# kamisli-icpl/LLICTI

Measured on AMD Instinct MI355X. Metric: MPix/s encode+decode, higher is better.
Workload: dtype f32; 1 GPU; 24x768x512 uniform-noise RGB per GPU, container xauto15 -> xrans20, seed-1337 weights; BASELINE.json configs[2]; batch_per_gpu=24, height=512, width=768, container=xauto15, container_written=xrans20

## Files before the change

__graft_entry__.py:

```python
import os
import subprocess
import sys

ROOT = os.path.dirname(os.path.abspath(__file__))
if ROOT not in sys.path:
    sys.path.insert(0, ROOT)


def build() -> None:
    from llicti_amd import _lib
    so = _lib.build()
    L = _lib.lib()
    assert L.llicti_version()
    _lib.build_probe()
    from oracle import oracle as orc
    orc.build()
    import llicti_amd
    from llicti_amd.graphs.models.LLICTI_nets import LLICTI
    from llicti_amd.agents.llicti_agent import LLICTIAgent
    print("built", so)


def smoke() -> None:
    import numpy as np
    import torch
    assert torch.cuda.is_available(), "smoke() needs cuda:0"
    from llicti_amd.codec import HipCodec, container_to_bytestream_list
    from llicti_amd.config import default_config
    from llicti_amd.graphs.models.LLICTI_nets import LLICTI
    from llicti_amd.weights import pack_state_dict
    from oracle import oracle as orc

    torch.manual_seed(1337)
    model = LLICTI(default_config()).to("cuda:0").eval()
    rgb = np.random.default_rng(0).integers(0, 256, size=(3, 96, 160), dtype=np.uint8)
    x = torch.from_numpy(rgb.astype(np.float32) / np.float32(255)).unsqueeze(0).to("cuda:0")
    bl, _ = model.compress(x)
    model.codec().poison_workspace()
    x_reco = model.decompres(bl, torch.device("cuda:0"))
    assert np.array_equal((x_reco * 255).round().to(torch.uint8).cpu().numpy()[0], rgb), "lossless round trip failed"
    ref = orc.encode_image(rgb, orc.Weights(pack_state_dict(model.state_dict())))
    assert ref == bl, "HIP bitstream differs from the CPU oracle"
    nbytes = sum(len(s) for row in bl for s in row)
    from llicti_amd.codec import MODE_RANS
    codec = model.codec()
    dev_rgb = torch.from_numpy(rgb[None]).to("cuda:0")
    W_o = orc.Weights(pack_state_dict(model.state_dict()))
    sizes = []
    for M, wide in ((10, 2), (10, 1), (8, 0)):
        mode = MODE_RANS(M, wide=wide)
        cont, seg = codec.encode(dev_rgb, mode=mode)
        codec.check()
        got = container_to_bytestream_list(cont[0].cpu().numpy(), seg[0].cpu().numpy())
        assert got == orc.encode_image_rans(rgb, W_o, M, wide), "HIP rANS container differs from the CPU oracle"
        codec.poison_workspace()
        rec = codec.decode(cont, seg, 96, 160, mode=mode)
        codec.check()
        assert torch.equal(rec, dev_rgb), "rANS container: lossless round trip failed"
        sizes.append(int(seg.sum().item()))
    from llicti_amd.codec import MODE_RANS_AUTO, name_of_mode
    cont, seg = codec.encode(dev_rgb, mode=MODE_RANS_AUTO(3))
    codec.check()
    picked = codec.container_modes(cont)[0]
    assert container_to_bytestream_list(cont[0].cpu().numpy(), seg[0].cpu().numpy()) == orc.encode_image_rans(rgb, W_o, 3, 2, auto=True), "auto stream count: HIP container differs from the CPU oracle"
    codec.poison_workspace()
    assert torch.equal(codec.decode(cont, seg, 96, 160, mode=picked), dev_rgb), "auto stream count: lossless round trip failed"
    codec.check()
    small = np.random.default_rng(1).integers(0, 256, size=(3, 67, 93), dtype=np.uint8)
    mode = MODE_RANS(2, wide=2)
    flat = torch.from_numpy(np.concatenate([rgb.reshape(-1), small.reshape(-1)])).to("cuda:0")
    cont, seg = codec.encode_v(flat, [96, 67], [160, 93], mode)
    codec.check()
    for b, img in enumerate((rgb, small)):
        assert container_to_bytestream_list(cont[b].cpu().numpy(), seg[b].cpu().numpy()) == orc.encode_image_rans(img, W_o, 2, 2), "mixed-size batch differs from the CPU oracle"
    codec.poison_workspace()
    assert torch.equal(codec.decode_v(cont, seg, [96, 67], [160, 93], mode), flat), "mixed-size batch: lossless round trip failed"
    codec.check()
    print(f"smoke ok: 96x160 image, {nbytes} bytes (reference format) / {sizes[0]} bytes (rANS, 10 xwide v4 streams) / {sizes[1]} bytes "
          f"(10 wide streams) / {sizes[2]} bytes (8 streams), xauto3 -> {name_of_mode(picked)}, and a 96x160 + 67x93 batch in one call: all bit-exact with the oracle, lossless")

if __name__ == "__main__":
    build()
    if len(sys.argv) > 1 and sys.argv[1] == "smoke":
        smoke()
```

llicti_amd/_lib.py:

```python
from __future__ import annotations

import ctypes as C
import os
import subprocess

_HERE = os.path.dirname(os.path.abspath(__file__))
ROOT = os.path.dirname(_HERE)
SO_PATH = os.environ.get("LLICTI_HIP_SO") or os.path.join(_HERE, "libllicti_hip.so")
_CSRC = os.path.join(_HERE, "csrc")
SOURCES = [os.path.join(_CSRC, "llicti_hip.hip")] + sorted(os.path.join(_CSRC, f) for f in os.listdir(_CSRC) if f.endswith(".hpp")) + \
          [os.path.join(ROOT, "include", "llicti_hip.h")]
HIPCC_FLAGS = ["--offload-arch=gfx950", "-O3", "-std=c++17", "-ffp-contract=off", "-fPIC", "-shared",
               "-Wno-unused-value"]

OK, EINVAL, EHIP, ENOWEIGHTS, ENOSPACE, EFORMAT, ENODEVICE = 0, -1, -2, -3, -4, -5, -6


class LlictiError(RuntimeError):
    def __init__(self, code, msg):
        super().__init__(f"llicti_hip error {code}: {msg}")
        self.code = code


def build(force: bool = False) -> str:
    stale = force or not os.path.exists(SO_PATH) or any(
        os.path.getmtime(s) > os.path.getmtime(SO_PATH) for s in SOURCES)
    if stale:
        hipcc = os.environ.get("HIPCC", "/opt/rocm/bin/hipcc")
        cmd = [hipcc] + HIPCC_FLAGS + ["-o", SO_PATH, SOURCES[0]]
        subprocess.check_call(cmd)
    return SO_PATH


PROBE_SRC = os.path.join(ROOT, "tests", "numerics_probe.hip")
PROBE_PATH = os.path.join(ROOT, "tests", "numerics_probe")


def build_probe(force: bool = False) -> str:
    deps = [PROBE_SRC, os.path.join(_CSRC, "numerics.hpp")]
    stale = force or not os.path.exists(PROBE_PATH) or any(os.path.getmtime(s) > os.path.getmtime(PROBE_PATH) for s in deps)
    if stale:
        hipcc = os.environ.get("HIPCC", "/opt/rocm/bin/hipcc")
        flags = [f for f in HIPCC_FLAGS if f not in ("-shared", "-fPIC")]
        subprocess.check_call([hipcc] + flags + ["-o", PROBE_PATH, PROBE_SRC])
    return PROBE_PATH


_lib = None
_vp, _i, _l, _sz =C.c_void_p, C.c_int, C.c_long, C.c_size_t
VIEW_GROUPS_MAX = 16
RECORD_CHUNK = 32768


class ViewGroup(C.Structure):
    _fields_ = [("d_out", C.c_void_p), ("dtype", C.c_int), ("Ho", C.c_int), ("Wo", C.c_int), ("antialias", C.c_int), ("n", C.c_int),
                ("image", C.c_void_p), ("y0", C.c_void_p), ("x0", C.c_void_p), ("hs", C.c_void_p), ("ws", C.c_void_p), ("flip", C.c_void_p)]


class TensorOpts(C.Structure):
    _fields_ = [("layout", C.c_int), ("pad_mode", C.c_int), ("fill_space", C.c_int), ("fill", C.c_float * 3)]


_SIGS = {
    "llicti_last_error": (C.c_char_p, []),
    "llicti_version": (C.c_char_p, []),
    "llicti_create": (_i, [C.POINTER(_vp), _i]),
    "llicti_destroy": (_i, [_vp]),
    "llicti_set_band_weights": (_i, [_vp, _i, _i] + [_vp] * 6),
    "llicti_set_model": (_i, [_vp, _i, _i]),
    "llicti_workspace_bytes_ctx": (_sz, [_vp, _i, _vp, _vp, _vp, _i]),
    "llicti_max_container_bytes_ctx": (_sz, [_vp, _i, _i]),
    "llicti_level_geom": (_i, [_i, _i, _i, _i] + [C.POINTER(_i)] * 8),
    "llicti_lift_u8": (_i, [_vp, _vp, _i, _i, _i, _vp, _vp, _vp, _vp]),
    "llicti_unlift_u8": (_i, [_vp, _vp, _i, _i, _i, _vp, _vp]),
    "llicti_band_params_f32": (_i, [_vp, _vp, _i, _i, _i, _i, _i, _vp, _vp]),
    "llicti_lift_train_f32": (_i, [_vp, _vp, _i, _i, _i, _vp, _vp]),
    "llicti_selfinfo_f32": (_i, [_vp, _vp, _vp, _i, _i, _i, _i, _i, _vp, _vp]),
    "llicti_cdf_u16": (_i, [_vp, _vp, _vp, _vp, _i, _i, _i, _i, _i, _i, _vp, _i, _vp]),
    "llicti_cdf_pairs_u32": (_i, [_vp, _vp, _vp, _vp, _i, _i, _i, _i, _i, _vp, _vp]),
    "llicti_ac_encode_u16cdf": (_i, [_vp, _vp, _i, _i, _vp, _i, _l, _vp, _l, _vp, _vp]),
    "llicti_ac_decode_u16cdf": (_i, [_vp, _vp, _i, _i, _vp, _l, _vp, _i, _l, _vp, _vp]),
    "llicti_workspace_bytes": (_sz, [_i, _i, _i, _i]),
    "llicti_workspace_bytes_v": (_sz, [_i, _vp, _vp, _i]),
    "llicti_workspace_bytes_vm": (_sz, [_i, _vp, _vp, _vp]),
    "llicti_encode_images_vm": (_i, [_vp, _vp, _vp, _i, _vp, _vp, _vp, _vp, _sz, _vp, _sz, _vp, _vp]),
    "llicti_decode_images_vm": (_i, [_vp, _vp, _sz, _vp, _i, _vp, _vp, _vp, _vp, _sz, _vp, _vp, _vp]),
    "llicti_encode_images_v": (_i, [_vp, _vp, _vp, _i, _vp, _vp, _i, _vp, _sz, _vp, _sz, _vp, _vp]),
    "llicti_decode_images_v": (_i, [_vp, _vp, _sz, _vp, _i, _vp, _vp, _i, _vp, _sz, _vp, _vp, _vp]),
    "llicti_reduced_dims": (_i, [_i, _i, _i, C.POINTER(_i), C.POINTER(_i)]),
    "llicti_decode_images_reduced": (_i, [_vp, _vp, _sz, _vp, _i, _vp, _vp, _vp, _i, _i, _vp, _sz, _vp, _vp, _vp]),
    "llicti_pixel_bytes": (_i, [_i]),
    "llicti_pixel_span": (_sz, [_i, _i, _i, _sz]),
    "llicti_encode_images_px": (_i, [_vp, _vp, _i, _vp, _vp, _i, _vp, _vp, _vp, _vp, _sz, _vp, _sz, _vp, _vp]),
    "llicti_decode_images_px": (_i, [_vp, _vp, _sz, _vp, _i, _vp, _vp, _vp, _i, _i, _vp, _sz, _vp, _i, _vp, _vp, _vp]),
    "llicti_tensor_elem_bytes": (_i, [_i]),
    "llicti_tensor_window_ok": (_i, [_i] * 7),
    "llicti_decode_images_tensor": (_i, [_vp, _vp, _sz, _vp, _i, _vp, _vp, _vp, _i, _i, _vp, _sz, _vp, _i, _i, _i, _vp, _vp, _vp, _vp, _vp, _vp]),
    "llicti_resize_window_ok": (_i, [_i] * 10),
    "llicti_resize_axis": (_i, [_i, _i, _i, _i, C.POINTER(_i), C.POINTER(C.c_float), _i]),
    "llicti_decode_images_tensor_resized": (_i, [_vp, _vp, _sz, _vp, _i, _vp, _vp, _vp, _i, _i, _vp, _sz, _vp, _i, _i, _i, _vp, _vp, _vp, _vp, _vp, _vp, _vp, _i, _vp]),
    "llicti_decode_images_tensor_views": (_i, [_vp, _vp, _sz, _vp, _i, _vp, _vp, _vp, _i, _i, _vp, _sz, C.POINTER(ViewGroup), _i, _vp, _vp, _vp]),
    "llicti_decode_images_reduced_rv": (_i, [_vp, _vp, _sz, _vp, _i, _vp, _vp, _vp, _i, _vp, _vp, _sz, _vp, _vp, _vp]),
    "llicti_decode_images_px_rv": (_i, [_vp, _vp, _sz, _vp, _i, _vp, _vp, _vp, _i, _vp, _vp, _sz, _vp, _i, _vp, _vp, _vp]),
    "llicti_decode_images_tensor_rv": (_i, [_vp, _vp, _sz, _vp, _i, _vp, _vp, _vp, _i, _vp, _vp, _sz, _vp, _i, _i, _i, _vp, _vp, _vp, _vp, _vp, _vp]),
    "llicti_decode_images_tensor_resized_rv": (_i, [_vp, _vp, _sz, _vp, _i, _vp, _vp, _vp, _i, _vp, _vp, _sz, _vp, _i, _i, _i, _vp, _vp, _vp, _vp, _vp, _vp, _vp, _i, _vp]),
    "llicti_decode_images_tensor_views_rv": (_i, [_vp, _vp, _sz, _vp, _i, _vp, _vp, _vp, _i, _vp, _vp, _sz, C.POINTER(ViewGroup), _i, _vp, _vp, _vp]),
    "llicti_pad_index": (_i, [_i] * 3),
    "llicti_tensor_window_pad_ok": (_i, [_i] * 8),
    "llicti_decode_images_tensor_o": (_i, [_vp, _vp, _sz, _vp, _i, _vp, _vp, _vp, _i, _vp, _vp, _sz, _vp, _i, _i, _i, _vp, _vp, _vp, _vp, _vp, _vp, C.POINTER(TensorOpts)]),
    "llicti_decode_images_tensor_resized_o": (_i, [_vp, _vp, _sz, _vp, _i, _vp, _vp, _vp, _i, _vp, _vp, _sz, _vp, _i, _i, _i, _vp, _vp, _vp, _vp, _vp, _vp, _vp, _i, _vp,
                                                   C.POINTER(TensorOpts)]),
    "llicti_decode_images_tensor_views_o": (_i, [_vp, _vp, _sz, _vp, _i, _vp, _vp, _vp, _i, _vp, _vp, _sz, C.POINTER(ViewGroup), _i, _vp, _vp, _vp, C.POINTER(TensorOpts)]),
    "llicti_encode_images_f32": (_i, [_vp, _vp, _vp, _i, _vp, _vp, _vp, _vp, _sz, _vp, _sz, _vp, _vp]),
    "llicti_max_container_bytes": (_sz, [_i, _i]),
    "llicti_transcode_workspace_bytes": (_sz, [_vp, _i, _vp, _vp, _vp, _i, _vp, _i]),
    "llicti_transcode_images": (_i, [_vp, _vp, _sz, _vp, _i, _vp, _vp, _vp, _i, _vp, _i, _vp, _sz, _vp, _sz, _vp, _vp]),
    "llicti_record_bytes": (_sz, [_vp, _vp]),
    "llicti_record_bytes_n": (_sz, [_i, _vp]),
    "llicti_pack_records": (_i, [_vp, _vp, _sz, _vp, _i, _vp, _sz, _vp, _vp]),
    "llicti_unpack_records": (_i, [_vp, _vp, _sz, _vp, _i, _vp, _sz, _vp, _vp]),
    "llicti_level_cuts": (_i, [_vp, _vp, _sz, _vp, _i, _vp, _vp, _vp, _vp, _sz, _vp, _vp]),
    "llicti_pack_progressive": (_i, [_vp, _vp, _sz, _vp, _i, _vp, _vp, _sz, _vp, _vp, _vp]),
    "llicti_unpack_progressive": (_i, [_vp, _vp, _sz, _vp, _i, _vp, _vp, _sz, _vp, _vp]),
    "llicti_progressive_prefix": (_i, [_vp, _sz, _vp]),
    "llicti_crc32_combine": (C.c_uint32, [C.c_uint32, C.c_uint32, C.c_uint64]),
    "llicti_crc32_geometry": (_i, [C.POINTER(_i), C.POINTER(_i)]),
    "llicti_crc32_planes": (_i, [_vp, _vp, _i, _i, _i, _vp, _vp]),
    "llicti_digest_images": (_i, [_vp, _i, _vp, _vp, _vp, _i, _vp, _vp, _sz, _vp, _vp, _vp]),
    "llicti_encode_images": (_i, [_vp, _vp, _i, _i, _i, _i, _vp, _sz, _vp, _sz, _vp, _vp]),
    "llicti_decode_images": (_i, [_vp, _vp, _sz, _vp, _i, _i, _i, _i, _vp, _sz, _vp, _vp]),
    "llicti_check_status": (_i, [_vp, _vp]),
    "llicti_header_dims": (_i, [_vp, C.POINTER(_i), C.POINTER(_i)]),
    "llicti_header_mode": (_i, [_vp, C.POINTER(_i)]),
    "llicti_image_status": (_i, [_vp, _vp, _i, _vp]),
    "llicti_selftest": (_i, []),
    "llicti_last_timing": (_i, [_vp, C.POINTER(C.c_float), C.POINTER(_i)]),
    "llicti_last_timing_detail": (_i, [_vp, C.POINTER(C.c_float), C.POINTER(C.c_float), _i, C.POINTER(_i)]),
    "llicti_last_cnn_level_ms": (_i, [_vp, C.POINTER(C.c_float)]),
    "llicti_set_profiling": (_i, [_vp, _i]),
    "llicti_get_counter": (_i, [_vp, C.c_char_p, C.POINTER(_l)]),
    "llicti_workspace_planes": (_i, [_vp, _i, _i, _i, _i, C.POINTER(_sz), C.POINTER(_sz)]),
    "llicti_workspace_params_v": (_i, [_vp, _i, _vp, _vp, _vp, _i, C.POINTER(_sz), C.POINTER(_l)]),
    "llicti_set_tuning": (_i, [_vp, C.c_char_p, _i]),
}
EXPORTS = sorted(_SIGS)


def lib():
    global _lib
    if _lib is None:
        import torch
        if not os.path.exists(SO_PATH):
            raise LlictiError(ENODEVICE, f"{SO_PATH} is missing: run __graft_entry__.build() (hipcc); "
                                         "there is no CPU fallback for the LLICTI hot path")
        L = C.CDLL(SO_PATH)
        for name, (res, args) in _SIGS.items():
            f = getattr(L, name)
            f.restype = res
            f.argtypes = args
        _lib = L
    return _lib


def check(rc: int):
    if rc != 0:
        raise LlictiError(rc, lib().llicti_last_error().decode(errors="replace"))


def level_geom(H, W, lvl, band=0):
    v = [_i() for _ in range(8)]
    check(lib().llicti_level_geom(H, W, lvl, band, *[C.byref(x) for x in v]))
    return tuple(x.value for x in v)


if __name__ == "__main__":
    print(build(force=True))
```

llicti_amd/csrc/rans_tail.hpp:

```cpp
#pragma once

#ifndef TAIL_AHEAD
#define TAIL_AHEAD 4
#endif
constexpr int kTailAhead = TAIL_AHEAD;

template <int Q> constexpr int kTailChains = kSeeded<Q> ? 2 : 1;
template <int Q> constexpr int tail_threads = 64 * (1 + kTailAhead) * kTailChains<Q>;

__device__ __forceinline__ int tail_lane() { return threadIdx.x & 63; }

template <int Q> struct RansTail {
    using GEO = RansGeo<Q>;
    static constexpr int L = 64 * Q, NCH = kTailChains<Q>;
    static constexpr int kSpillDw = kSeeded<Q> ? kRansSpillMax / 32 + 1 : 0;
    static constexpr int kArenaDw = GEO::kPayDw + kSpillDw;
    static constexpr int NSL = NCH * kTailAhead;
    const float *params; const uint32_t *rstate; int16_t *planes; float *fplanes; int32_t *status; const uint8_t *slots; const long *rslot_off;
    uint32_t *sh_pay;
    float (*sh_cmp)[NSL][16];
    int (*sh_e1)[NSL][64];
    long (*sh_off)[NSL];
    int (*sh_spec)[NSL][16];
    int *sh_cur;
    int sidx, b, m, M;
    StageGeom sg; int nc, cnt;
    Grid gr; int max_symbol, shift; uint32_t pw;
    int alen;
    SeededTailShape shape;
    int wave, role, chain;
    bool pool, live; int SA, T, R;
    bool bad;
    struct Pos { int pi, pj; };
    __device__ __forceinline__ Pos pos(int j) const {
        const int q = min(max(cnt - 1 - j, 0), max(cnt - 1, 0));
        const int n = min(rans_stream_pos(q, m, M, L), nc - 1);
        const int pi = div_wc(sg, n), pj = n - pi * sg.wc;
        return Pos{ pi, pj };
    }
    __device__ __forceinline__ long pixel_off(int pi, int pj) const { return sg.img_off + ((long)(2 * pi + sg.oi) << sg.lvl) * sg.W + ((long)(2 * pj + sg.oj) << sg.lvl); }
    __device__ __forceinline__ void store_pixel(long off, int v) const {
        planes[off + 2 * sg.plane] = (int16_t)v;
        fplanes[off + 2 * sg.plane] = div255_exact((float)v);
    }
};

template <int Q> __device__ __forceinline__ void tail_open(RansTail<Q> &t, const StageGeom *sgv, const StreamRef *sref, const uint32_t *rpos,
                                                           const uint32_t *rtail, const int32_t *minmax, const int *act)
{
    using TL = RansTail<Q>;
    t.sidx = act ? act[blockIdx.x] : (int)blockIdx.x;
    const StreamRef sr_ = sref[t.sidx];
    t.b = sr_.b; t.m = sr_.m; t.M = sr_.M;
    t.wave = __builtin_amdgcn_readfirstlane((int)(threadIdx.x >> 6));
    t.role = t.wave / TL::NCH;
    t.sg = sgv[t.b];
    t.nc = t.sg.hc * t.sg.wc;
    t.cnt = rans_stream_count(t.nc, t.m, t.M, TL::L);
    const int rt = (int)(rtail[t.sidx] & 0xFFFFu);
    const int nch = (kSeeded<Q> && !(rtail[t.sidx] >> 16)) ? 2 : 1;
    t.pool = TL::NCH == 2 && nch == 1;
    t.chain = (t.pool && t.role != 0) ? 0 : t.wave % TL::NCH;
    t.SA = t.pool ? TL::NSL : kTailAhead;
    const int E = kSeeded<Q> ? (int)rpos[t.sidx] : 0;
    t.bad = (kSeeded<Q> ? E >= kRansSpillMax : rpos[t.sidx] != 0) || rt > t.cnt;
    t.alen = TL::GEO::kPayBits + (t.bad ? 0 : E);
    const int Tall = min(rt, t.cnt);
    int minv, maxv;
    clr_range(minmax + 4 * t.b, 2, minv, maxv, t.shift);
    t.gr = make_grid(minv, maxv);
    t.max_symbol = t.gr.Lp - 2;
    t.pw = 1;
    const int ns = kSeeded<Q> ? rans_seed_count(t.max_symbol + 1, t.pw) : 0;
    t.shape = seeded_tail_shape(t.cnt, Tall, nch, ns, kSeeded<Q>);
    t.bad = t.bad || Tall < t.shape.NS || (nch == 2 && t.cnt < 2 * ns);
    t.live = t.chain < nch;
    t.T = t.live ? t.shape.chain_count(t.chain) : 0;
    t.R = (t.shape.chain_count(0) + t.SA - 1) / t.SA;
}

__device__ __forceinline__ uint32_t tail_window_entry(const Grid &gr, int max_symbol, int we, float wn, float mu, float rsig, int idx)
{
    const float pt = sample_pt(gr, min(idx, gr.Lp - 1));
    const float term = mix_term(wn, mu, rsig, pt);
    const int g0 = 4 * 5 * min(we, 11);
    const float a0 = __int_as_float(__builtin_amdgcn_ds_bpermute(g0, __float_as_int(term)));
    const float a1 = __int_as_float(__builtin_amdgcn_ds_bpermute(g0 + 4, __float_as_int(term)));
    const float a2 = __int_as_float(__builtin_amdgcn_ds_bpermute(g0 + 8, __float_as_int(term)));
    const float a3 = __int_as_float(__builtin_amdgcn_ds_bpermute(g0 + 12, __float_as_int(term)));
    const float a4 = __int_as_float(__builtin_amdgcn_ds_bpermute(g0 + 16, __float_as_int(term)));
    const float acc = (((a0 + a1) + a2) + a3) + a4;
    return (idx <= max_symbol) ? entry_from_sum(acc, gr.scale, idx) : 0x10000u;
}

template <int Q> __device__ __forceinline__ void tail_prepare_role(const RansTail<Q> &t)
{
    using TL = RansTail<Q>;
    const int lane = tail_lane(), mc = lane % 5, we = lane / 5, max_symbol = t.max_symbol, SA = t.SA, T = t.T;
    const StageGeom &sg = t.sg;
    const Grid &gr = t.gr;
    const int i = t.pool ? t.wave - TL::NCH : t.role - 1;
    const int sl = t.chain * kTailAhead + i;
    struct Row { float sg, mu, wk, bb, dd, y, co; long off; };
    auto fetch = [&](int k) -> Row {
        Row r;
        const auto pp = t.pos(t.shape.index(t.chain, T - 1 - k));
        const int pi = pp.pi, pj = pp.pj;
        const ParRow src = par_row(t.params + sg.par_off, 0, (long)sg.h * sg.w, (long)pi * sg.w + pj);
        r.off = t.pixel_off(pi, pj);
        r.sg = src[10 + mc]; r.mu = src[16 + 10 + mc]; r.wk = src[32 + 10 + mc];
        r.bb = src[48 + 5 + mc]; r.dd = src[48 + 10 + mc];
        r.y = t.fplanes[r.off]; r.co = t.fplanes[r.off + sg.plane];
        return r;
    };
    auto prepare = [&](const Row &row, int buf) {
        const float t1 = row.bb * row.y;
        const float t2 = row.dd * row.co;
        const float tt = t1 + t2;
        const float mu = row.mu + tt;
        const float rsig = 1.0f / mix_sigma(row.sg);
        const float w = (row.wk > kWeightBound) ? row.wk : kWeightBound;
        float wk5[5], mu5[5], rs5[5];
#pragma unroll
        for (int k = 0; k < 5; ++k) wk5[k] = __int_as_float(__builtin_amdgcn_readlane(__float_as_int(w), k));
        const float wn = w / mix_weight_den(wk5[0], wk5[1], wk5[2], wk5[3], wk5[4]);
#pragma unroll
        for (int k = 0; k < 5; ++k) {
            mu5[k] = __int_as_float(__builtin_amdgcn_readlane(__float_as_int(mu), k));
            rs5[k] = __int_as_float(__builtin_amdgcn_readlane(__float_as_int(rsig), k));
            wk5[k] = __int_as_float(__builtin_amdgcn_readlane(__float_as_int(wn), k));
        }
        const int i1 = min(8 * lane, max_symbol);
        const float pt1 = sample_pt(gr, i1);
        float sum = 0.0f;
#pragma unroll
        for (int k = 0; k < 5; ++k) { Comp ck; ck.mu = mu5[k]; ck.rsig = rs5[k]; ck.wn = wk5[k]; sum += term_fast(comp_fast(ck), pt1); }
        const int e1v = (int)__builtin_rintf(sum * gr.scale) + i1;
        t.sh_e1[buf][sl][lane] = e1v;
        if (lane < 5) { t.sh_cmp[buf][sl][lane] = mu; t.sh_cmp[buf][sl][5 + lane] = rsig; t.sh_cmp[buf][sl][10 + lane] = wn; }
        if (lane == 0) t.sh_off[buf][sl] = row.off;
        const int lst = __builtin_amdgcn_readfirstlane(__builtin_popcountll(ballot64(lane == 0 || (8 * lane <= max_symbol && e1v <= 0x8000))) - 1);
        const int eL = __builtin_amdgcn_readlane(e1v, lst);
        const int eH = (lst < 63 && 8 * (lst + 1) <= max_symbol) ? __builtin_amdgcn_readlane(e1v, min(lst + 1, 63)) : 0x10000;
        int wbs = -1;
        if (eH - eL >= 0x2000) {
            const float fr = 8.0f * (float)(0x8000 - eL) * __builtin_amdgcn_rcpf((float)(eH - eL));
            wbs = max(8 * lst + (int)__builtin_amdgcn_fmed3f(fr, 0.0f, 8.0f) - 5, 0);
            const uint32_t ent = tail_window_entry(gr, max_symbol, we, wn, mu, rsig, wbs + min(we, 11));
            if (mc == 0 && we < 12) t.sh_spec[buf][sl][we] = (int)ent;
        }
        if (lane == 0) t.sh_spec[buf][sl][12] = wbs;
    };
    Row rowA = fetch(i);
    Row rowB = fetch(SA + i);
    prepare(rowA, 0);
    __syncthreads();
    __syncthreads();
    for (int r = 0; r < t.R; ++r) {
        const Row rowC = fetch(SA * (r + 2) + i);
        if (SA * (r + 1) + i < T) prepare(rowB, (r + 1) & 1);
        rowB = rowC;
        lds_barrier();
    }
    if constexpr (kSeeded<Q>) lds_barrier();
}

template <int Q> __device__ __forceinline__ void tail_assemble(const RansTail<Q> &t)
{
    using TL = RansTail<Q>;
    const int lane = tail_lane();
    uint32_t *const sh_pay = t.sh_pay;
#pragma unroll
    for (int qq = 0; qq < Q; ++qq) sh_pay[64 * qq + lane] = 0;
    if (lane < 2) sh_pay[64 * Q + lane] = 0;
    __builtin_amdgcn_wave_barrier();
#pragma unroll
    for (int qq = 0; qq < Q; ++qq) {
        const uint32_t xl = t.rstate[((long)t.sidx * Q + qq) * 64 + lane] & 0x7FFFFFFFu;
        lds_or_bits(sh_pay, kRansStateBits * (64 * qq + lane), 16, xl & 0xFFFFu);
        lds_or_bits(sh_pay, kRansStateBits * (64 * qq + lane) + 16, kRansStateBits - 16, xl >> 16);
    }
    if constexpr (kSeeded<Q>) {
        if (lane < TL::kSpillDw) {
            const uint32_t w = reinterpret_cast<const uint32_t *>(t.slots + t.rslot_off[t.sidx] + 4)[lane];
            const int nb = min(max(t.alen - TL::GEO::kPayBits - 32 * lane, 0), 32);
            sh_pay[TL::GEO::kPayDw + lane] = nb >= 32 ? w : (w & ((1u << nb) - 1u));
        }
    }
}

struct TailCoder { uint32_t xt; int tc, a_end; };

template <int Q> __device__ __forceinline__ TailCoder tail_start_state(RansTail<Q> &t)
{
    using TL = RansTail<Q>;
    const int lane = tail_lane(), alen = t.alen;
    const uint32_t *const sh_pay = t.sh_pay;
    TailCoder c;
    c.a_end = alen;
    if constexpr (kSeeded<Q>) {
        c.xt = !t.live ? (1u << 31) : (uint32_t)__builtin_amdgcn_readfirstlane((int)(t.chain ? lds_get_bits(sh_pay, alen - 32, 32) : sh_pay[0]));
        c.tc = t.chain ? alen - (t.live ? 32 : 0) : 32;
        if (t.shape.nch == 2) { if (!(c.xt >> 31)) { t.bad = true; c.xt |= 1u << 31; } }
        else {
            int top = -1;
            for (int d0 = 64 * ((TL::kArenaDw - 1) / 64); d0 >= 0 && top < 0; d0 -= 64) {
                const int d = d0 + lane;
                const uint32_t w = (d >= 1 && d < TL::kArenaDw) ? sh_pay[d] : 0u;
                const uint64_t nz = ballot64(w != 0);
                if (nz) {
                    const int hl = 63 - __clzll((long long)nz);
                    top = 32 * (d0 + hl) + 31 - __clz((int)__builtin_amdgcn_readlane((int)w, hl));
                }
            }
            if (top < 32 || (alen > TL::GEO::kPayBits && top != alen - 1)) { t.bad = true; top = 32; }
            c.a_end = top;
        }
    } else {
        int top = -1;
#pragma unroll
        for (int qq = Q - 1; qq >= 0; --qq) {
            const uint64_t nz = ballot64(sh_pay[64 * qq + lane] != 0);
            if (top < 0 && nz) {
                const int hd = 64 * qq + 63 - __clzll((long long)nz);
                top = 32 * hd + 31 - __clz((int)sh_pay[hd]);
            }
        }
        if (top < 31) t.bad = true;
        c.xt = (top >= 31) ? (uint32_t)__builtin_amdgcn_readfirstlane((int)lds_get_bits(sh_pay, top - 31, 32)) : (1u << 31);
        c.tc = (top >= 31) ? top - 31 : 0;
    }
    return c;
}

struct TailBits {
    uint32_t w0, w1; int base;
    __device__ __forceinline__ uint32_t bits(int pos, int n) const { return (uint32_t)((((uint64_t)w1 << 32) | w0) >> (pos - base)) & ((1u << n) - 1u); }
};
__device__ __forceinline__ int tail_clamp_bits(int nb, int avail, bool &bad)
{
    if (nb > 16 || avail < nb) { bad = true; nb = max(min(nb, min(avail, 16)), 0); }
    return nb;
}
__device__ __forceinline__ void tail_take_down(TailCoder &c, const TailBits &w, int nb) { c.tc -= nb; c.xt = (c.xt << nb) | w.bits(c.tc, nb); }
__device__ __forceinline__ void tail_take_up(TailCoder &c, const TailBits &w, int nb) { c.xt = (c.xt << nb) | w.bits(c.tc, nb); c.tc += nb; }

template <int Q> __device__ __forceinline__ void tail_renorm(RansTail<Q> &t, TailCoder &c, const TailBits &w, bool first_coded, uint32_t freq)
{
    if constexpr (kSeeded<Q>) {
        int nb = __clz((int)c.xt);
        if (t.shape.nch == 2) {
            nb = tail_clamp_bits(nb, t.chain ? c.tc - 32 : t.alen - 32 - c.tc, t.bad);
            if (t.chain) tail_take_down(c, w, nb); else tail_take_up(c, w, nb);
            c.xt |= 1u << 31;
        } else {
            const int avail = c.a_end - c.tc;
            if (nb > avail) nb = max(avail, 0);
            tail_take_up(c, w, tail_clamp_bits(nb, 16, t.bad));
        }
    } else if (first_coded) t.bad = t.bad || c.xt != freq << 15;
    else {
        tail_take_down(c, w, tail_clamp_bits(__clz((int)c.xt), c.tc, t.bad));
        c.xt |= 1u << 31;
    }
}

template <int Q> __device__ __forceinline__ void tail_decode_rounds(RansTail<Q> &t, TailCoder &c)
{
    const int lane = tail_lane(), mc = lane % 5, we = lane / 5, max_symbol = t.max_symbol, SA = t.SA, T = t.T;
    for (int r = 0; r < t.R; ++r) {
        const int buf = r & 1;
        int vsym = 0;
        for (int i = 0; i < SA && SA * r + i < T; ++i) {
            const int sl = t.chain * kTailAhead + i;
            const uint32_t slot = c.xt & 0xFFFFu;
            const int wv = t.sh_spec[buf][sl][min(lane, 12)];
            const bool up = kSeeded<Q> && t.chain == 0;
            const int wpos = min(max(up ? c.tc : c.tc - 16, 0), t.alen);
            const TailBits bw{ (uint32_t)__builtin_amdgcn_readfirstlane((int)t.sh_pay[wpos >> 5]),
                               (uint32_t)__builtin_amdgcn_readfirstlane((int)t.sh_pay[(wpos >> 5) + 1]), wpos & ~31 };
            int wb = __builtin_amdgcn_readlane(wv, 12), np = 0;
            if (wb >= 0) np = __builtin_popcountll((ballot64((uint32_t)wv <= slot) & 0xFFFull) | (wb == 0 ? 1ull : 0ull));
            uint32_t vlo, vhi;
            if (np >= 1 && np <= 11) {
                vlo = (uint32_t)__builtin_amdgcn_readlane(wv, np - 1);
                vhi = (uint32_t)__builtin_amdgcn_readlane(wv, np);
            } else {
                const float mu = t.sh_cmp[buf][sl][mc], rsig = t.sh_cmp[buf][sl][5 + mc], wn = t.sh_cmp[buf][sl][10 + mc];
                const int e1 = t.sh_e1[buf][sl][lane];
                auto entry_at = [&](int idx) -> uint32_t { return tail_window_entry(t.gr, max_symbol, we, wn, mu, rsig, idx); };
                const uint64_t p1 = ballot64(lane == 0 || (8 * lane <= max_symbol && e1 <= (int)slot));
                wb = max(8 * (__builtin_popcountll(p1) - 1) - 2, 0);
                uint32_t ent = entry_at(wb + we);
                const uint64_t pw12 = ballot64(mc == 0 && we < 12 && wb + we <= max_symbol && (ent <= slot || wb + we == 0));
                np = __builtin_popcountll(pw12);
                if (np == 0 || np == 12) {
                    int lo = 0, hi = max_symbol + 1;
                    while (hi - lo > 1) {
                        const int stp = (hi - lo + 12) / 13;
                        const int pi = min(lo + stp * (min(we, 11) + 1), hi - 1);
                        const uint32_t e = entry_at(pi);
                        const uint64_t pb = ballot64(mc == 0 && we < 12 && e <= slot);
                        const int k = __builtin_popcountll(pb);
                        const int nlo = (k > 0) ? min(lo + stp * k, hi - 1) : lo;
                        const int nhi = (k < 12) ? min(lo + stp * (k + 1), hi - 1) : hi;
                        lo = nlo; hi = nhi;
                    }
                    wb = lo;
                    ent = entry_at(wb + we);
                    np = 1;
                }
                vlo = (uint32_t)__builtin_amdgcn_readlane((int)ent, 5 * (np - 1));
                vhi = (uint32_t)__builtin_amdgcn_readlane((int)ent, 5 * np);
            }
            vsym = (lane == i) ? wb + np - 1 - t.shift : vsym;
            c.xt = (vhi - vlo) * (c.xt >> 16) + slot - vlo;
            tail_renorm(t, c, bw, SA * r + i == T - 1, vhi - vlo);
        }
        if (lane < SA && SA * r + lane < T) t.store_pixel(t.sh_off[buf][t.chain * kTailAhead + lane], vsym);
        lds_barrier();
    }
}

template <int Q> __device__ __forceinline__ void tail_finish(RansTail<Q> &t, const TailCoder &c)
{
    using TL = RansTail<Q>;
    const int lane = tail_lane();
    bool bad = t.bad;
    if constexpr (kSeeded<Q>) {
        const int nch = t.shape.nch, sn = t.shape.sn;
        const uint32_t A = (uint32_t)(t.max_symbol + 1), v = (nch == 2) ? (c.xt & 0x7FFFFFFFu) : c.xt;
        bad = bad || (t.live && (nch == 2 ? v >= t.pw : (v >= A || c.tc != c.a_end)));
        uint32_t div = 1;
        for (int e = 0; e < min(lane, sn); ++e) div *= A;
        const int dg = (lane < sn) ? (int)((v / div) % A) : 0;
        const int j = t.shape.seed_index(t.chain, lane);
        if (t.live && lane < sn && j < t.shape.NS) {
            const auto pp = t.pos(j);
            t.store_pixel(t.pixel_off(pp.pi, pp.pj), dg - t.shift);
        }
        bad = bad || ballot64(t.live && lane < sn && j >= t.shape.NS && dg != 0) != 0;
        if (lane == 0) t.sh_cur[t.chain] = c.tc;
        lds_barrier();
        if (t.chain == 0 && nch == 2) {
            const int ca = t.sh_cur[0], cb = t.sh_cur[1];
            uint32_t nz = 0;
            for (int d = lane; d < TL::kArenaDw; d += 64) {
                const int lo = max(ca, 32 * d), hi = min(cb, 32 * d + 32);
                if (lo < hi) nz |= t.sh_pay[d] & ((hi - lo == 32) ? 0xFFFFFFFFu : (((1u << (hi - lo)) - 1u) << (lo - 32 * d)));
            }
            bad = bad || ca > cb || ballot64(nz != 0) != 0;
        }
        if (bad && lane == 0) flag_image(t.status, t.b, LLICTI_EFORMAT);
    } else {
        if (t.T == 0) bad = bad || c.xt != (1u << 31);
        if ((bad || c.tc != 0) && lane == 0) flag_image(t.status, t.b, LLICTI_EFORMAT);
    }
}

template <int Q>
__global__ __launch_bounds__(tail_threads<Q>) void rans_tail_kernel(const float *__restrict__ params, const StageGeom *__restrict__ sgv, const StreamRef *__restrict__ sref,
                                                       const uint32_t *__restrict__ rstate, const uint32_t *__restrict__ rpos,
                                                       const uint32_t *__restrict__ rtail,
                                                       int16_t *__restrict__ planes, float *__restrict__ fplanes,
                                                       const int32_t *__restrict__ minmax, int32_t *status,
                                                       const uint8_t *__restrict__ slots, const long *__restrict__ rslot_off,
                                                       const int *__restrict__ act = nullptr)
{
    using TL = RansTail<Q>;
    __shared__ uint32_t sh_pay[64 * Q + 2 + TL::kSpillDw];
    __shared__ float sh_cmp[2][TL::NSL][16];
    __shared__ int sh_e1[2][TL::NSL][64];
    __shared__ long sh_off[2][TL::NSL];
    __shared__ int sh_spec[2][TL::NSL][16];
    __shared__ int sh_cur[2];
    TL t{ params, rstate, planes, fplanes, status, slots, rslot_off, sh_pay, sh_cmp, sh_e1, sh_off, sh_spec, sh_cur };
    tail_open(t, sgv, sref, rpos, rtail, minmax, act);
    if (t.role != 0) tail_prepare_role(t);
    else {
        if (t.wave == 0) tail_assemble(t);
        __syncthreads();
        TailCoder c = tail_start_state(t);
        __syncthreads();
        tail_decode_rounds(t, c);
        tail_finish(t, c);
    }
}
```

Measured before the change: 451.3 MPix/s.

## Replace ds_bpermute mixture sums with DPP row-shift group sums in rANS tail decode

Remaps the tail coder's lanes so that each 5-component mixture sum lives inside one 16-lane DPP row, and computes the sum with a chain of row-shift DPP adds instead of five ds_bpermute cross-lane gathers. The sum result now sits on the mc==4 lane, and a lookup helper finds that lane when reading out entries. The change also moves the payload LDS loads earlier so they overlap the symbol search, and raises wave priority during the decode rounds. This trades LDS-routed permutes for cheaper in-register DPP ops, but it relies on an intricate lane mapping that has to stay bit-exact. It also adds a new probe build step.

Result: no change. 451.2 MPix/s, median of 3 (-0.0%).

```diff
diff --git a/__graft_entry__.py b/__graft_entry__.py
--- a/__graft_entry__.py
+++ b/__graft_entry__.py
@@ -13,6 +13,7 @@
     L = _lib.lib()
     assert L.llicti_version()
     _lib.build_probe()
+    _lib.build_group_sum_probe()
     from oracle import oracle as orc
     orc.build()
     import llicti_amd
diff --git a/llicti_amd/_lib.py b/llicti_amd/_lib.py
--- a/llicti_amd/_lib.py
+++ b/llicti_amd/_lib.py
@@ -44,6 +44,20 @@
         flags = [f for f in HIPCC_FLAGS if f not in ("-shared", "-fPIC")]
         subprocess.check_call([hipcc] + flags + ["-o", PROBE_PATH, PROBE_SRC])
     return PROBE_PATH
+
+
+GROUP_SUM_SRC = os.path.join(ROOT, "tests", "group_sum_probe.hip")
+GROUP_SUM_PATH = os.path.join(ROOT, "tests", "group_sum_probe")
+
+
+def build_group_sum_probe(force: bool = False) -> str:
+    deps = [GROUP_SUM_SRC] + SOURCES[1:]
+    stale = force or not os.path.exists(GROUP_SUM_PATH) or any(os.path.getmtime(s) > os.path.getmtime(GROUP_SUM_PATH) for s in deps)
+    if stale:
+        hipcc = os.environ.get("HIPCC", "/opt/rocm/bin/hipcc")
+        flags = [f for f in HIPCC_FLAGS if f not in ("-shared", "-fPIC")]
+        subprocess.check_call([hipcc] + flags + ["-o", GROUP_SUM_PATH, GROUP_SUM_SRC])
+    return GROUP_SUM_PATH
 
 
 _lib = None
diff --git a/llicti_amd/csrc/rans_tail.hpp b/llicti_amd/csrc/rans_tail.hpp
--- a/llicti_amd/csrc/rans_tail.hpp
+++ b/llicti_amd/csrc/rans_tail.hpp
@@ -79,24 +79,30 @@
     t.R = (t.shape.chain_count(0) + t.SA - 1) / t.SA;
 }
 
-__device__ __forceinline__ uint32_t tail_window_entry(const Grid &gr, int max_symbol, int we, float wn, float mu, float rsig, int idx)
+__device__ __forceinline__ int tail_lane_mc(int lane) { return (lane & 15) % 5; }
+__device__ __forceinline__ int tail_lane_entry(int lane) { return min(3 * (lane >> 4) + (lane & 15) / 5, 11); }
+__device__ __forceinline__ bool tail_lane_is_sum(int mc) { return mc == 4; }
+__device__ __forceinline__ int tail_sum_lane(int e) { return (e << 2) + e + 4 + ((0xFEA540 >> (e << 1)) & 3); }
+
+__device__ __forceinline__ float tail_group_sum(float term)
+{
+    float s = term;
+#pragma unroll
+    for (int k = 0; k < 4; ++k) s = __int_as_float(__builtin_amdgcn_update_dpp(0, __float_as_int(s), 0x111, 0xF, 0xF, true)) + term;
+    return s;
+}
+
+__device__ __forceinline__ uint32_t tail_window_entry(const Grid &gr, int max_symbol, float wn, float mu, float rsig, int idx)
 {
     const float pt = sample_pt(gr, min(idx, gr.Lp - 1));
-    const float term = mix_term(wn, mu, rsig, pt);
-    const int g0 = 4 * 5 * min(we, 11);
-    const float a0 = __int_as_float(__builtin_amdgcn_ds_bpermute(g0, __float_as_int(term)));
-    const float a1 = __int_as_float(__builtin_amdgcn_ds_bpermute(g0 + 4, __float_as_int(term)));
-    const float a2 = __int_as_float(__builtin_amdgcn_ds_bpermute(g0 + 8, __float_as_int(term)));
-    const float a3 = __int_as_float(__builtin_amdgcn_ds_bpermute(g0 + 12, __float_as_int(term)));
-    const float a4 = __int_as_float(__builtin_amdgcn_ds_bpermute(g0 + 16, __float_as_int(term)));
-    const float acc = (((a0 + a1) + a2) + a3) + a4;
+    const float acc = tail_group_sum(mix_term(wn, mu, rsig, pt));
     return (idx <= max_symbol) ? entry_from_sum(acc, gr.scale, idx) : 0x10000u;
 }
 
 template <int Q> __device__ __forceinline__ void tail_prepare_role(const RansTail<Q> &t)
 {
     using TL = RansTail<Q>;
-    const int lane = tail_lane(), mc = lane % 5, we = lane / 5, max_symbol = t.max_symbol, SA = t.SA, T = t.T;
+    const int lane = tail_lane(), mc = tail_lane_mc(lane), we = tail_lane_entry(lane), max_symbol = t.max_symbol, SA = t.SA, T = t.T;
     const StageGeom &sg = t.sg;
     const Grid &gr = t.gr;
     const int i = t.pool ? t.wave - TL::NCH : t.role - 1;
@@ -146,8 +152,8 @@
         if (eH - eL >= 0x2000) {
             const float fr = 8.0f * (float)(0x8000 - eL) * __builtin_amdgcn_rcpf((float)(eH - eL));
             wbs = max(8 * lst + (int)__builtin_amdgcn_fmed3f(fr, 0.0f, 8.0f) - 5, 0);
-            const uint32_t ent = tail_window_entry(gr, max_symbol, we, wn, mu, rsig, wbs + min(we, 11));
-            if (mc == 0 && we < 12) t.sh_spec[buf][sl][we] = (int)ent;
+            const uint32_t ent = tail_window_entry(gr, max_symbol, wn, mu, rsig, wbs + we);
+            if (tail_lane_is_sum(mc)) t.sh_spec[buf][sl][we] = (int)ent;
         }
         if (lane == 0) t.sh_spec[buf][sl][12] = wbs;
     };
@@ -267,18 +273,19 @@
 
 template <int Q> __device__ __forceinline__ void tail_decode_rounds(RansTail<Q> &t, TailCoder &c)
 {
-    const int lane = tail_lane(), mc = lane % 5, we = lane / 5, max_symbol = t.max_symbol, SA = t.SA, T = t.T;
+    const int lane = tail_lane(), mc = tail_lane_mc(lane), we = tail_lane_entry(lane), max_symbol = t.max_symbol, SA = t.SA, T = t.T;
+    const bool sum_lane = tail_lane_is_sum(mc);
+    __builtin_amdgcn_s_setprio(3);
     for (int r = 0; r < t.R; ++r) {
-        const int buf = r & 1;
+        const int buf = r & 1, sl0 = t.chain * kTailAhead;
         int vsym = 0;
         for (int i = 0; i < SA && SA * r + i < T; ++i) {
-            const int sl = t.chain * kTailAhead + i;
+            const int sl = sl0 + i;
+            const int wv = t.sh_spec[buf][sl][min(lane, 12)];
             const uint32_t slot = c.xt & 0xFFFFu;
-            const int wv = t.sh_spec[buf][sl][min(lane, 12)];
             const bool up = kSeeded<Q> && t.chain == 0;
             const int wpos = min(max(up ? c.tc : c.tc - 16, 0), t.alen);
-            const TailBits bw{ (uint32_t)__builtin_amdgcn_readfirstlane((int)t.sh_pay[wpos >> 5]),
-                               (uint32_t)__builtin_amdgcn_readfirstlane((int)t.sh_pay[(wpos >> 5) + 1]), wpos & ~31 };
+            const uint32_t pay0 = t.sh_pay[wpos >> 5], pay1 = t.sh_pay[(wpos >> 5) + 1];
             int wb = __builtin_amdgcn_readlane(wv, 12), np = 0;
             if (wb >= 0) np = __builtin_popcountll((ballot64((uint32_t)wv <= slot) & 0xFFFull) | (wb == 0 ? 1ull : 0ull));
             uint32_t vlo, vhi;
@@ -288,19 +295,19 @@
             } else {
                 const float mu = t.sh_cmp[buf][sl][mc], rsig = t.sh_cmp[buf][sl][5 + mc], wn = t.sh_cmp[buf][sl][10 + mc];
                 const int e1 = t.sh_e1[buf][sl][lane];
-                auto entry_at = [&](int idx) -> uint32_t { return tail_window_entry(t.gr, max_symbol, we, wn, mu, rsig, idx); };
+                auto entry_at = [&](int idx) -> uint32_t { return tail_window_entry(t.gr, max_symbol, wn, mu, rsig, idx); };
                 const uint64_t p1 = ballot64(lane == 0 || (8 * lane <= max_symbol && e1 <= (int)slot));
                 wb = max(8 * (__builtin_popcountll(p1) - 1) - 2, 0);
                 uint32_t ent = entry_at(wb + we);
-                const uint64_t pw12 = ballot64(mc == 0 && we < 12 && wb + we <= max_symbol && (ent <= slot || wb + we == 0));
+                const uint64_t pw12 = ballot64(sum_lane && wb + we <= max_symbol && (ent <= slot || wb + we == 0));
                 np = __builtin_popcountll(pw12);
                 if (np == 0 || np == 12) {
                     int lo = 0, hi = max_symbol + 1;
                     while (hi - lo > 1) {
                         const int stp = (hi - lo + 12) / 13;
-                        const int pi = min(lo + stp * (min(we, 11) + 1), hi - 1);
+                        const int pi = min(lo + stp * (we + 1), hi - 1);
                         const uint32_t e = entry_at(pi);
-                        const uint64_t pb = ballot64(mc == 0 && we < 12 && e <= slot);
+                        const uint64_t pb = ballot64(sum_lane && e <= slot);
                         const int k = __builtin_popcountll(pb);
                         const int nlo = (k > 0) ? min(lo + stp * k, hi - 1) : lo;
                         const int nhi = (k < 12) ? min(lo + stp * (k + 1), hi - 1) : hi;
@@ -310,16 +317,19 @@
                     ent = entry_at(wb + we);
                     np = 1;
                 }
-                vlo = (uint32_t)__builtin_amdgcn_readlane((int)ent, 5 * (np - 1));
-                vhi = (uint32_t)__builtin_amdgcn_readlane((int)ent, 5 * np);
+                const int nu = __builtin_amdgcn_readfirstlane(np);
+                vlo = (uint32_t)__builtin_amdgcn_readlane((int)ent, tail_sum_lane(nu - 1));
+                vhi = (uint32_t)__builtin_amdgcn_readlane((int)ent, tail_sum_lane(nu));
             }
             vsym = (lane == i) ? wb + np - 1 - t.shift : vsym;
             c.xt = (vhi - vlo) * (c.xt >> 16) + slot - vlo;
+            const TailBits bw{ (uint32_t)__builtin_amdgcn_readfirstlane((int)pay0), (uint32_t)__builtin_amdgcn_readfirstlane((int)pay1), wpos & ~31 };
             tail_renorm(t, c, bw, SA * r + i == T - 1, vhi - vlo);
         }
-        if (lane < SA && SA * r + lane < T) t.store_pixel(t.sh_off[buf][t.chain * kTailAhead + lane], vsym);
+        if (lane < SA && SA * r + lane < T) t.store_pixel(t.sh_off[buf][sl0 + lane], vsym);
         lds_barrier();
     }
+    __builtin_amdgcn_s_setprio(0);
 }
 
 template <int Q> __device__ __forceinline__ void tail_finish(RansTail<Q> &t, const TailCoder &c)
```
